# lucianpls/QB3

Measured on AMD Instinct MI355X. Metric: MPixel/s encode+decode (QB3M_FTL, 8-bit 3-band), higher is better.
Workload: dtype u8; 1 GPU; 16384x16384x3 uint8 NOISY3 seed 2; QB3M_FTL qb3x_encode_device (self-indexed container, table level 2) + qb3x_decode_device of that container alone (index = NULL, restart table inside the container); table_level=2, container_bytes=458870207

## Files before the change

qb3_amd/csrc/api_mem.cpp:

```cpp
#include <chrono>
#include <mutex>
#include "qb3_host.h"

using namespace qb3dev;
using namespace qb3api;

struct DevPool {
    struct Item { void *p; size_t cap; int dev; };
    static constexpr size_t POOL_ITEMS = 24;
    const size_t POOL_BYTES = [] { const char *e = getenv("QB3_POOL_MB"); return (e && e[0] ? (size_t)strtoull(e, nullptr, 10) : (size_t)3072) << 20; }();
    std::mutex mu;
    std::vector<Item> items;
    size_t bytes = 0;
    void *take(size_t n, int dev, size_t *cap) {
        std::lock_guard<std::mutex> l(mu);
        size_t best = items.size();
        for (size_t i = 0; i < items.size(); i++)
            if (items[i].dev == dev && items[i].cap >= n && items[i].cap / 2 <= n && (best == items.size() || items[i].cap < items[best].cap)) best = i;
        if (best == items.size()) return nullptr;
        void *p = items[best].p;
        *cap = items[best].cap;
        bytes -= items[best].cap;
        items.erase(items.begin() + (long)best);
        return p;
// ... 46 lines not shown
    bool any = false;
    for (DevBuf *b : bufs) any = any || b->p != nullptr;
    if (any) (void)hipDeviceSynchronize();
    for (DevBuf *b : bufs) b->release(true);
}
QB3_API void qb3x_trim(void) { try { dev_pool().trim(); qb3host::ring_trim(); } catch (...) {} }

bool qb3api::device_ok() {
    int n = 0;
    hipError_t e = hipGetDeviceCount(&n);
    if (e != hipSuccess || n <= 0) { set_error("no usable HIP device (the block codec has no CPU fallback)", (int)e); return false; }
    return true;
}

hipError_t qb3api::wait_stream(hipStream_t st) {
    const auto t0 = std::chrono::steady_clock::now();
    for (uint32_t i = 0;; i++) {
        const hipError_t e = hipStreamQuery(st);
        if (e != hipErrorNotReady) return e;
        if ((i & 63) == 63 && std::chrono::steady_clock::now() - t0 > std::chrono::milliseconds(4)) break;
    }
    return hipStreamSynchronize(st);
}
hipError_t qb3api::fetch_small(void *dst, const void *d_src, size_t n, hipStream_t st) {
    static thread_local void *pinned = nullptr;
    if (!pinned && hipHostMalloc(&pinned, 1024, hipHostMallocDefault) != hipSuccess) pinned = nullptr;
    if (!pinned || n > 1024) {
        hipError_t e = hipMemcpyAsync(dst, d_src, n, hipMemcpyDeviceToHost, st);
        return e == hipSuccess ? hipStreamSynchronize(st) : e;
    }
    hipError_t e = hipMemcpyAsync(pinned, d_src, n, hipMemcpyDeviceToHost, st);
    if (e == hipSuccess) e = wait_stream(st);
    if (e == hipSuccess) memcpy(dst, pinned, n);
    return e;
}

static void parallel_memcpy(uint8_t *dst, const uint8_t *src, size_t n) {
    try { qb3host::CopyPool::get().copy(dst, src, n); }
    catch (...) { memcpy(dst, src, n); }
}
bool qb3api::upload(Stager &sg, void *d_dst, const void *h_src, size_t bytes, hipStream_t st) {
    if (bytes < Stager::MIN_BYTES || !sg.init()) {
        hipError_t e = hipMemcpyAsync(d_dst, h_src, bytes, hipMemcpyHostToDevice, st);
        if (e != hipSuccess) { set_error("upload", (int)e); return false; }
        return true;
    }
    size_t i = 0;
    for (size_t off = 0; off < bytes; off += Stager::SLICE, i++) {
        const size_t n = std::min(Stager::SLICE, bytes - off);
        if (i >= Stager::NSLOT && hipEventSynchronize(sg.ev(i)) != hipSuccess) { set_error("upload: slot wait", 0); return false; }
// ... 60 lines not shown
```

qb3_amd/csrc/api_tiles.cpp:

```cpp
#include "qb3_host.h"

using namespace qb3dev;
using namespace qb3api;

static size_t encode_tiles_loop(encsp p, const void *d_src, size_t first, size_t n, size_t src_pitch, void *d_dst, size_t dst_pitch,
                                void *d_index, size_t isz, size_t *sizes, void *stream, qb3_mode mode) {
    size_t done = 0;
    for (size_t i = first; i < first + n; i++) {
        qb3_reset_encoder(p);
        p->mode = mode;
        sizes[i] = qb3x_encode_device(p, (const uint8_t *)d_src + i * src_pitch, (uint8_t *)d_dst + i * dst_pitch,
                                      d_index ? (uint8_t *)d_index + i * isz : nullptr, stream);
        done += sizes[i] != 0;
    }
    return done;
}

static size_t encode_tiles_body(encsp p, const void *d_src, size_t n, size_t src_pitch, void *d_dst, size_t dst_pitch,
                                void *d_index, size_t *sizes, void *stream) {
    if (!p || !d_src || !d_dst || !sizes || (dst_pitch & 3) || ((uintptr_t)d_dst & 3)) return 0;
    const size_t isz = d_index ? qb3x_index_size(p) : 0;
    const qb3_mode mode = p->mode;
    const size_t tsz = szof(p->type);
    hipStream_t st = (hipStream_t)stream;
    const bool batchable = !is_rle_mode(mode) && mode != QB3M_STORED && p->quanta < 2 && p->xsize >= 4 && p->ysize >= 4 &&
                           p->xsize * p->ysize > 16 && !p->error && device_ok();
    if (!batchable) {
        const size_t k = encode_tiles_loop(p, d_src, 0, n, src_pitch, d_dst, dst_pitch, d_index, isz, sizes, stream, mode);
        if (mode != QB3M_STORED) p->mode = mode;
        return k;
    }

    uint8_t hdrbuf[80];
    size_t hdr = write_headers(p, hdrbuf);
    Geometry g = make_geometry(p->xsize, p->ysize, p->nbands, p->type, p->stride, p->order, p->mode, p->cband, nullptr);
    EncPlan plan = plan_encode(g);
    size_t wsp = (plan.ws_bytes + 255) & ~(size_t)255;
    size_t batch = (size_t)8 << 30 >= wsp ? ((size_t)8 << 30) / wsp : 1;
    if (batch > n) batch = n;
    if (batch > 65535) batch = 65535;
    if (!p->d_ws.ensure(batch * wsp)) { p->error = QB3E_LIBERR; return 0; }
    IxTable ixt;
    size_t hdr_stamp = hdr, ix_bytes = 0, isz_all = isz;
    void *index_all = d_index;
    if (ix_room(p)) {
        ixt = ix_layout(g, p->ix_chunk);
        hdr_stamp = write_headers(p, hdrbuf, false);
// ... 163 lines not shown
```

qb3_amd/csrc/k_enc_post.hip:

```cpp
#include "qb3_kernels.h"
#include "qb3_ix_fill.h"

namespace qb3dev {

__global__ void __launch_bounds__(SCAN_GROUP / 4) enc_scan_kernel(const EncArgs a0) {
    const EncArgs a = enc_for_tile(a0, blockIdx.y);
    __shared__ uint32_t wsum[16];
    __shared__ uint64_t wsum64[16];
    __shared__ uint64_t carry;
    __shared__ uint32_t is_last;
    const uint32_t tid = threadIdx.x, i0 = blockIdx.x * SCAN_GROUP + 4 * tid;
    const uint32_t ngroups = (a.nchunks + SCAN_GROUP - 1) / SCAN_GROUP;
    uint32_t v[4], sum = 0;
#pragma unroll
    for (int k = 0; k < 4; k++) { v[k] = (i0 + k < a.nchunks) ? a.chunk_bits[i0 + k] : 0; sum += v[k]; }
    uint32_t total;
    uint64_t off = block_exscan(sum, wsum, &total);
#pragma unroll
    for (int k = 0; k < 4; k++) if (i0 + k < a.nchunks) { a.chunk_off[i0 + k] = off; off += v[k]; }
    if (tid == 0) {
        a.group_sum[blockIdx.x] = total;
        __threadfence();
        is_last = atomicAdd((uint32_t *)&a.group_sum[ngroups + 1], 1u) == gridDim.x - 1;
        carry = 0;
    }
    __syncthreads();
    if (!is_last) return;
    __threadfence();
    for (uint32_t base = 0; base < ngroups; base += blockDim.x) {
        const uint32_t i = base + tid;
        const uint64_t g = i < ngroups ? __hip_atomic_load(&a.group_sum[i], __ATOMIC_RELAXED, __HIP_MEMORY_SCOPE_AGENT) : 0ull;
        const uint64_t ex = block_exscan_v<uint64_t>(g, wsum64);
        const uint64_t c0 = carry;
        if (i < ngroups) a.group_sum[i] = c0 + ex;
        __syncthreads();
        if (tid == blockDim.x - 1) carry = c0 + ex + g;
        __syncthreads();
    }
    if (tid == 0) { a.group_sum[ngroups] = carry; a.res->zero_run = 0; a.res->ff_pairs = 0; a.res->zero_dwords = 0; }
}

__device__ __forceinline__ uint64_t chunk_start(const EncArgs &a, uint32_t k) {
    if (k >= a.nchunks) return a.group_sum[(a.nchunks + SCAN_GROUP - 1) / SCAN_GROUP];
    return a.group_sum[k / SCAN_GROUP] + a.chunk_off[k];
}

__device__ __forceinline__ uint32_t zero_runs_in(uint32_t cur, uint32_t nxt) {
    return (uint32_t)(cur == 0) + (uint32_t)(__builtin_amdgcn_alignbit(nxt, cur, 8) == 0) +
           (uint32_t)(__builtin_amdgcn_alignbit(nxt, cur, 16) == 0) + (uint32_t)(__builtin_amdgcn_alignbit(nxt, cur, 24) == 0);
}
__device__ __forceinline__ uint32_t ff_pairs_in(uint32_t v) {
    const uint32_t t = v & (v >> 8) & 0x00ffffffu;
    return (uint32_t)__popc(((t & 0x7f7f7fu) + 0x010101u) & t & 0x808080u);
}

__device__ __forceinline__ void ix_finish_chunk(const EncArgs &a, uint32_t c) {
    typedef uint32_t u32_a1 __attribute__((aligned(1)));
    __shared__ uint32_t part[4];
    const uint32_t tid = threadIdx.x;
    const uint32_t here = (a.ix_K - c * a.ix_per_chunk < a.ix_per_chunk) ? a.ix_K - c * a.ix_per_chunk : a.ix_per_chunk;
    uint8_t *chunk = a.ix_dst + (uint64_t)c * (IX_HEAD + IX_PAD + (uint64_t)a.ix_per_chunk * a.ix_E);
    uint8_t *e0 = chunk + IX_HEAD;
// ... 318 lines not shown
```

qb3_amd/csrc/k_host.hip:

```cpp
#include "qb3_kernels.h"
#include "qb3_walk.h"

namespace qb3dev {

static thread_local char g_err[256] = "";
const char *last_error() { return g_err; }
void set_error(const char *what, int e) {
    snprintf(g_err, sizeof(g_err), "%s: %s", what, e ? hipGetErrorString((hipError_t)e) : "failed");
}

const Tuning &tuning() {
    static const Tuning t = [] {
        auto on = [](const char *name) { const char *e = getenv(name); return e && e[0] && e[0] != '0'; };
        Tuning v;
        v.no_px = on("QB3_NO_PX");
        v.slow_walk = on("QB3_SLOW_WALK");
        const char *cap = getenv("QB3_WALK_TAB_KB");
        v.walk_tab_kb = cap ? (size_t)strtoull(cap, nullptr, 10) : 0;
        v.slow_index = on("QB3_SLOW_INDEX");
        { const char *e = getenv("QB3_WIDE_BAND"); v.wide_band = e && e[0] ? atoi(e) : 0; }
        v.no_bl = on("QB3_NO_BLOCK_LENGTHS");
        { const char *e = getenv("QB3_BEST_SAMPLE_MIN"); v.best_sample_min = e && e[0] ? (uint32_t)strtoul(e, nullptr, 10) : BEST_SAMPLE_MIN; }
        { const char *e = getenv("QB3_EXITS_FROM"); v.exits_from = e && e[0] ? (int64_t)strtoll(e, nullptr, 10) : -1; }
        return v;
    }();
    return t;
}

}
#include <map>
#include <mutex>
#include <string>
#include <vector>
namespace qb3dev {
struct ProfPending { const char *name; hipEvent_t a, b; };
static std::mutex g_prof_mu;
static int g_prof_level = 0;
static std::vector<ProfPending> g_prof_pending;
static std::vector<hipEvent_t> g_prof_pool;
static std::map<std::string, std::pair<double, uint64_t>> g_prof_acc;
void prof_enable(int level) { std::lock_guard<std::mutex> l(g_prof_mu); g_prof_level = level; }
static bool prof_minor(const char *n) { const std::string s(n); return s == "enc_scan" || s == "enc_seams" || s == "enc_best_scan" || s == "enc_best_recode"; }
void prof_reset() { std::lock_guard<std::mutex> l(g_prof_mu); g_prof_acc.clear(); }
static hipEvent_t prof_event() {
    if (!g_prof_pool.empty()) { hipEvent_t e = g_prof_pool.back(); g_prof_pool.pop_back(); return e; }
    hipEvent_t e = nullptr;
    (void)hipEventCreate(&e);
    return e;
}
ProfScope::ProfScope(const char *n, hipStream_t s) : st(s), name(n) {
    std::lock_guard<std::mutex> l(g_prof_mu);
    on = g_prof_level == 1 || (g_prof_level == 2 && !prof_minor(n)) || (g_prof_level >= 3 && std::string(n).find("_units") != std::string::npos);
    if (on) { a = prof_event(); b = prof_event(); (void)hipEventRecord(a, st); }
}
ProfScope::~ProfScope() {
    if (!on) return;
    (void)hipEventRecord(b, st);
    std::lock_guard<std::mutex> l(g_prof_mu);
    g_prof_pending.push_back({name, a, b});
}
void prof_collect() {
    std::lock_guard<std::mutex> l(g_prof_mu);
    std::vector<ProfPending> keep;
    for (auto &p : g_prof_pending) {
        float ms = 0;
        const hipError_t e = hipEventElapsedTime(&ms, p.a, p.b);
        if (e == hipErrorNotReady) { keep.push_back(p); continue; }
        if (e == hipSuccess) { auto &acc = g_prof_acc[p.name]; acc.first += ms; acc.second++; }
        g_prof_pool.push_back(p.a); g_prof_pool.push_back(p.b);
    }
    (void)hipGetLastError();
    g_prof_pending.swap(keep);
}
bool prof_get(const char *name, double *total_ms, uint64_t *count) {
    std::lock_guard<std::mutex> l(g_prof_mu);
    auto it = g_prof_acc.find(name);
    if (it == g_prof_acc.end()) return false;
    *total_ms = it->second.first; *count = it->second.second;
    return true;
}
int prof_names(char *buf, size_t n) {
    std::lock_guard<std::mutex> l(g_prof_mu);
    std::string s;
    for (auto &kv : g_prof_acc) { if (!s.empty()) s += ","; s += kv.first; }
    snprintf(buf, n, "%s", s.c_str());
    return (int)g_prof_acc.size();
}


static void fast_geometry(uint32_t bands, uint32_t tsz, uint32_t *threads, uint32_t *bpp, uint32_t *passes) {
    *threads = tsz == 8 ? 128 : 256;
    *bpp = *threads / bands;
    uint32_t k = (uint32_t)(16384 / ((size_t)*bpp * bands * tsz * 16));
    *passes = k < 1 ? 1 : (k > 3 ? 3 : k);
}
static void px16_split(const Geometry &g, uint32_t *bg, uint32_t *ng) {
    const uint32_t B = g.bands;
    *bg = B <= 4 ? B : (B % 4 == 0) ? 4 : (B % 2 == 0) ? 2 : 0;
    *ng = *bg ? B / *bg : 0;
}
uint32_t px16_bands_per_lane(const Geometry &g) { uint32_t bg, ng; px16_split(g, &bg, &ng); return bg; }

uint32_t seg_blocks_for(const Geometry &g) {
    if (lane_per_unit_shape(g.tsz, g.mode, g.bands)) return 64 / g.bands;
    if (g.mode != CM_BEST) {
// ... 175 lines not shown
}

static void launch_enc_units(const EncArgs &a, const EncPlan &plan, hipStream_t st) {
    if (a.g.mode == CM_BEST) { if (plan.px && a.g.tsz == 1) launch_enc_px_best(a, plan, st); else launch_enc_best(a, plan, st); }
    else if (plan.px && a.g.tsz == 1) {
        ProfScope ps("enc_units", st);
        launch_enc_px(a, plan, st);
    }
    else if (plan.px16 && a.g.tsz == 2 && ((uintptr_t)a.img & 1) == 0) { ProfScope ps("enc_units", st); launch_enc_px16(a, plan, st); }
    else if (plan.pxw && ((uintptr_t)a.img & (a.g.tsz - 1)) == 0 && !(a.ts_img & (a.g.tsz - 1))) { ProfScope ps("enc_units", st); launch_enc_pxw(a, plan, st); }
    else { ProfScope ps("enc_units", st); launch_enc_generic(a, plan, st); }
}
static int launch_encode_all(const EncArgs &a, const EncPlan &plan, hipStream_t st) {
    launch_enc_units(a, plan, st);
    launch_enc_post(a, plan, st);
    HIPCHK(hipGetLastError());
    return 0;
}

static bool make_enc_args(EncArgs &a, const Geometry &g, const EncPlan &plan, const void *img, uint32_t *out32, uint32_t out_bit0,
                          const BandState &st_in, void *ws, void *index, const TileBatch &tb,
                          const uint8_t *hdr, uint32_t hdr_len, const IxTable &ix, bool zrun_probe) {
    a.zrun_probe = zrun_probe ? 1u : 0u;
    a.ix_dst = ix.base; a.ix_K = ix.K; a.ix_E = ix.entry_bytes; a.ix_per_chunk = ix.per_chunk; a.ix_blocks = ix.blocks;
    a.ix_spe = g.seg_blocks ? ix.blocks / g.seg_blocks : 0;
    a.ntiles = tb.n ? tb.n : 1; a.ts_img = tb.src_pitch; a.ts_out = tb.dst_pitch; a.ts_ws = tb.ws_pitch; a.ts_idx = tb.idx_pitch;
    a.hdr_len = hdr_len <= sizeof(a.hdr) ? hdr_len : 0;
    a.hdr_back = a.hdr_len + (ix.base ? (uint32_t)ix_total_bytes(ix) + 2 : 0);
    for (uint32_t i = 0; i < a.hdr_len; i++) a.hdr[i] = hdr[i];
    a.g = g; a.img = img; a.out32 = out32; a.out_bit0 = out_bit0;
    a.slots = plan.slots; a.nchunks = plan.nchunks; a.dpr = g.bands * g.tsz;
    a.chunk0 = 0; a.chunk_end = plan.nchunks; a.finish_what = 3;
    a.magic_dpr = magic_div(a.dpr); a.magic_bands = magic_div(g.bands);
    uint8_t *w = (uint8_t *)ws;
    const EncWs L = enc_ws_layout(g, plan.nchunks, plan.nbp, plan.threads);
    a.chunk_bits = (uint32_t *)(w + L.bits);
    a.chunk_off = (uint64_t *)(w + L.off);
    a.group_sum = (uint64_t *)(w + L.gsum);
    a.seams = (uint32_t *)(w + L.seams);
    a.scratch = (uint32_t *)(w + L.scratch);
    a.cw_has = w + L.cwhas; a.cw_val = (uint64_t *)(w + L.cwval); a.centry = (uint64_t *)(w + L.centry); a.centry_parts = (uint32_t *)(w + L.cparts); a.recode_n = a.centry_parts + 32 * MAXBANDS;
    a.cw_used = w + L.cwused; a.seg_from_entry = w + L.segfe; a.recode_need = (uint32_t *)(w + L.rneed); a.recode_list = (uint32_t *)(w + L.rlist);
    a.slot_dw = L.slot_dw;
    a.px_ng = plan.px16 ? plan.px16_ng : 1; a.px_magic_ng = magic_div(a.px_ng);
    a.px16_bg = g.tsz == 2 ? px16_bands_per_lane(g) : 0;
    a.px_aligned = !(g.w & 3) && !((g.stride * g.tsz) & 3) && !((uintptr_t)img & 3) && !(tb.src_pitch & 3);
    a.res = (EncResult *)(w + L.res);
    a.st = st_in;
    a.ix_bl = ix.base && ix.block_lens;
    a.ix_coder = a.ix_bl && plan.px && g.tsz == 1 && g.mode != CM_BEST && g.seg_blocks == 64 && ix.blocks == 64;
    a.ix_wgs = 0;
    a.have_idx = index != nullptr && !(a.ix_coder && ix.own_index);
    a.idx_no_ulen = index && ix.base && ix.own_index && !ix.block_lens;
    a.idx = index ? index_view(g, index) : IndexView{nullptr, nullptr, nullptr, nullptr, nullptr};
    if (g.tsz != 1 && g.tsz != 2 && g.tsz != 4 && g.tsz != 8) { set_error("encode: bad value size", 0); return false; }
    return true;
}

int launch_encode(const Geometry &g, const EncPlan &plan, const void *img, uint32_t *out32, uint32_t out_bit0,
                  const BandState &st_in, void *ws, void *index, void *stream, const TileBatch &tb,
                  const uint8_t *hdr, uint32_t hdr_len, const IxTable &ix, bool zrun_probe) {
    EncArgs a;
    if (!make_enc_args(a, g, plan, img, out32, out_bit0, st_in, ws, index, tb, hdr, hdr_len, ix, zrun_probe)) return -1;
    return launch_encode_all(a, plan, (hipStream_t)stream);
}

bool encode_strips_ok(const Geometry &g, const EncPlan &plan) { return g.mode != CM_BEST && plan.nchunks > 2 * SCAN_GROUP; }
uint32_t encode_strip_count(const EncPlan &plan) { return (plan.nchunks + SCAN_GROUP - 1) / SCAN_GROUP; }
uint64_t encode_strip_blocks(const EncPlan &plan, uint32_t strip) {
    const uint64_t c = std::min<uint64_t>(plan.nchunks, ((uint64_t)strip + 1) * SCAN_GROUP);
    return c * plan.nbp;
}
const uint64_t *encode_strip_total(const Geometry &g, const EncPlan &plan, void *ws, uint32_t strip) {
    const EncWs L = enc_ws_layout(g, plan.nchunks, plan.nbp, plan.threads);
    return (const uint64_t *)((uint8_t *)ws + L.gsum) + strip + 1;
}
int launch_encode_strip(const Geometry &g, const EncPlan &plan, const void *img, uint32_t *out32, uint32_t out_bit0,
                        const BandState &st_in, void *ws, void *index, void *stream, const uint8_t *hdr, uint32_t hdr_len, const IxTable &ix, uint32_t strip) {
    EncArgs a;
    if (!make_enc_args(a, g, plan, img, out32, out_bit0, st_in, ws, index, TileBatch(), hdr, hdr_len, ix, false)) return -1;
    a.chunk0 = strip * SCAN_GROUP;
    a.chunk_end = std::min<uint32_t>(plan.nchunks, a.chunk0 + SCAN_GROUP);
    a.finish_what = 1;
    hipStream_t st = (hipStream_t)stream;
    launch_enc_units(a, plan, st);
    launch_enc_post_strip(a, plan, st, strip);
// ... 152 lines not shown
```

qb3_amd/csrc/qb3_api.cpp:

```cpp
#include <chrono>
#include <new>
#include <limits>
#include <thread>
#include "qb3_host.h"

using namespace qb3dev;
using namespace qb3api;

static size_t raw_size(const encs *p) { return p->xsize * p->ysize * p->nbands * szof(p->type); }

static CodecMode codec_mode(int mode) {
    if (mode == QB3M_FTL) return CM_FTL;
    if (mode == QB3M_BASE_H || mode == QB3M_BASE_Z || mode == QB3M_RLE || mode == QB3M_RLE_H) return CM_BASE;
    return CM_BEST;
}

Geometry qb3api::make_geometry(size_t w, size_t h, size_t bands, int dtype, size_t stride, uint64_t order, int mode,
                              const size_t *cband_sz, const uint8_t *cband_u8) {
    Geometry g;
    memset(&g, 0, sizeof(g));
    g.w = (uint32_t)w; g.h = (uint32_t)h; g.bands = (uint32_t)bands; g.tsz = (uint32_t)szof(dtype);
    g.stride = stride ? stride : w * bands;
    g.order = order ? order : HILBERT;
    g.nbx = (uint32_t)((w + 3) / 4); g.nby = (uint32_t)((h + 3) / 4);
// ... 87 lines not shown
    if (w < 4) {
        for (size_t y = 0; y < h; y++, d += w * pix) memcpy(d, src + y * stride_bytes, w * pix);
        nw = 4; nh = ngroups * 4;
    } else {
        for (size_t x = 0; x < w; x++)
            for (size_t y = 0; y < h; y++, d += pix) memcpy(d, src + y * stride_bytes + x * pix, pix);
        nw = ngroups * 4; nh = 4;
    }
    return t;
}


static size_t stored_encode_host(encsp p, const void *source, void *destination) {
    uint8_t *d = (uint8_t *)destination;
    p->mode = QB3M_STORED;
    const size_t hdr = write_headers(p, d);
    if (p->error) return 0;
    const size_t tsz = szof(p->type), line = p->xsize * p->nbands * tsz;
    const size_t stride = (p->stride ? p->stride : p->xsize * p->nbands) * tsz;
    for (size_t y = 0; y < p->ysize; y++) memcpy(d + hdr + y * line, (const uint8_t *)source + y * stride, line);
    return hdr + raw_size(p);
}

static bool encode_blocks_device(encsp p, const Geometry &g, const void *d_img, uint8_t *d_out, size_t hdr,
                                 void *d_index, hipStream_t st, bool carry, uint64_t *bits, const uint8_t *hdrbytes,
                                 size_t hdr_stamp, const IxTable &ix, int *zero_run = nullptr) {
    EncPlan plan = plan_encode(g);
    if (!p->d_ws.ensure(plan.ws_bytes)) return false;
    BandState bs;
    memset(&bs, 0, sizeof(bs));
    for (size_t c = 0; c < p->nbands; c++) {
        bs.prev[c] = p->band[c].prev; bs.cf[c] = p->band[c].cf; bs.rung[c] = (uint8_t)p->band[c].runbits;
    }
    uint32_t *out32 = (uint32_t *)(d_out + (hdr & ~(size_t)3));
    EncResult res;
    const uint8_t *dres = (const uint8_t *)p->d_ws.p + plan.ws_bytes - sizeof(EncResult);
    if (launch_encode(g, plan, d_img, out32, (uint32_t)(8 * (hdr & 3)), bs, p->d_ws.p, d_index, st, TileBatch(), hdrbytes, (uint32_t)hdr_stamp, ix, zero_run != nullptr)) return false;
    const hipError_t e = fetch_small(&res, dres, sizeof(res), st);
    if (e != hipSuccess) { set_error("encode kernels", (int)e); return false; }
    prof_collect();
    *bits = res.total_bits;
    { static const bool dbg = getenv("QB3_DEBUG_RLE") != nullptr; if (dbg && zero_run) fprintf(stderr, "encode: zero_run %llu ff_pairs %llu zero_dwords %llu (%u chunks)\n", (unsigned long long)res.zero_run, (unsigned long long)res.ff_pairs, (unsigned long long)res.zero_dwords, plan.nchunks); }
    if (zero_run) *zero_run = rle0_may_win(res) ? (rle0_no_uniform_chunk(res, (uint64_t)plan.nbp * g.bands / 4) ? 2 : 1) : 0;
    if (carry)
        for (size_t c = 0; c < p->nbands; c++) {
            p->band[c].prev = (size_t)res.prev[c]; p->band[c].runbits = res.rung[c]; p->band[c].cf = (size_t)res.cf[c];
        }
    return true;
}

struct ModeGuard {
    encs *p; qb3_mode mode; bool armed = true;
    ModeGuard(encs *h) : p(h), mode(h->mode) {}
    ~ModeGuard() { if (armed) p->mode = mode; }
};


static int encode_pipelined(encsp p, const Geometry &g, const void *host_src, void *host_dst, size_t src_bytes, size_t line, uint8_t *out_dev, size_t hdr,
                            const uint8_t *hdrbuf, size_t hdr_stamp, const IxTable &ixt, void *d_index, bool carry, uint64_t *bits_out) {
    using qb3host::CopyPool;
    constexpr size_t SLICE = Stager::SLICE, NSLOT = Stager::NSLOT;
    static const bool dbg = getenv("QB3_DEBUG_PIPE") != nullptr;
// ... 87 lines not shown
            if (q == hipSuccess) { if (dbg && !dn_copy) t_first_dn = ms_since(); pool.submit(dn[dn_copy].host, r2.slot(dn_copy), dn[dn_copy].n, b_dn[dn_copy % NSLOT]); dn_copy++; progress = true; }
            else if (q != hipErrorNotReady) e = q;
        }
        while (dn_freed < dn_copy && pool.done(b_dn[dn_freed % NSLOT])) { dn_freed++; progress = true; }
        if (!progress && !pool.help_one()) std::this_thread::yield();
    }
    (void)hipGetLastError();
    for (size_t i = 0; i < NSLOT; i++) { pool.wait(b_up[i]); pool.wait(b_dn[i]); }
    p->pipe.sync();
    if (dbg) fprintf(stderr, "encode_pipelined: setup %.2f ms, last upload enqueued %.2f, first slice down %.2f, done %.2f (%u strips, %zu + %zu slices)\n", t_setup, t_up_done, t_first_dn, ms_since(), nstrips, n_up, dn.size());
    if (!ok()) { if (!launch_failed) set_error("pipelined encode", (int)e); p->error = QB3E_LIBERR; return -1; }
    prof_collect();
    *bits_out = res_host->total_bits;
    if (carry)
        for (size_t c = 0; c < p->nbands; c++) {
            p->band[c].prev = (size_t)res_host->prev[c]; p->band[c].runbits = res_host->rung[c]; p->band[c].cf = (size_t)res_host->cf[c];
        }
    return 1;
}

static size_t encode_common(encsp p, const void *host_src, void *host_dst, const void *d_src, void *d_dst,
                            void *d_index, hipStream_t st) {
    const bool on_host = host_src != nullptr;
    const size_t tsz = szof(p->type), line = p->xsize * p->nbands * tsz;
    const size_t src_stride_bytes = (p->stride ? p->stride : p->xsize * p->nbands) * tsz;
    const size_t src_span = src_stride_bytes * (p->ysize - 1) + line;
    if (p->xsize * p->ysize <= 16) {
        if (on_host) return stored_encode_host(p, host_src, host_dst);
        std::vector<uint8_t> tmp(src_span), out(64 + raw_size(p));
        if (!device_ok()) { p->error = QB3E_LIBERR; return 0; }
        HIPOK(hipMemcpyAsync(tmp.data(), d_src, tmp.size(), hipMemcpyDeviceToHost, st));
        HIPOK(hipStreamSynchronize(st));
        size_t n = stored_encode_host(p, tmp.data(), out.data());
        HIPOK(hipMemcpyAsync(d_dst, out.data(), n, hipMemcpyHostToDevice, st));
        HIPOK(hipStreamSynchronize(st));
        return n;
    }
    ModeGuard guard(p);
    const qb3_mode mode = p->mode;
    const bool rle = is_rle_mode(mode);
    const size_t ixroom = mode == QB3M_STORED ? 0 : ix_room(p);
    if (rle) p->mode = (qb3_mode)((int)mode - 2);
    uint8_t hdrbuf[80];
    size_t hdr = write_headers(p, hdrbuf);
    if (p->error) return 0;
    if (!device_ok()) { p->error = QB3E_LIBERR; return 0; }
// ... 44 lines not shown

    IxTable ixt;
    size_t hdr_stamp = hdr;
    if (ixroom && !narrow) {
        ixt = ix_layout(g, p->ix_chunk);
        hdr_stamp = write_headers(p, hdrbuf, false);
        hdr = hdr_stamp + ix_total_bytes(ixt) + 2;
        ixt.base = out_dev + hdr_stamp;
        if (!d_index) {
            if (!p->d_idx.ensure(index_bytes(g))) { p->error = QB3E_LIBERR; return 0; }
            d_index = p->d_idx.p;
            ixt.own_index = true;
        }
    }
    uint64_t bits = 0;
    int has_run = 1;
    bool piped = false;
    if (want_pipe) {
        const int r = encode_pipelined(p, g, host_src, host_dst, src_span, line, out_dev, hdr, hdrbuf, hdr_stamp, ixt, d_index, carry, &bits);
        if (r < 0) return 0;
        piped = r > 0;
        if (!piped && !upload_now()) { p->error = QB3E_LIBERR; return 0; }
    }
    if (!piped && !encode_blocks_device(p, g, img_dev, out_dev, hdr, d_index, st, carry, &bits, hdrbuf, hdr_stamp, ixt, rle ? &has_run : nullptr)) {
        p->error = QB3E_LIBERR; return 0;
    }
    p->error = 0;
    const size_t len = hdr + (size_t)((bits + 7) / 8);
    const size_t len_ref = len - (ixt.base ? ix_total_bytes(ixt) : 0);

    if (rle) {
        p->mode = mode;
        if (len_ref <= maxsz / 2 && has_run) {
            const size_t n = len - hdr;
            uint64_t rsz64 = 0;
            if (!p->d_rle.ensure(rle0_ws_bytes(n)) || rle0_device_size(out_dev + hdr, n, p->d_rle.p, false, &rsz64, st, has_run == 2)) { p->error = QB3E_LIBERR; return 0; }
            const size_t rsz = (size_t)rsz64;
            if (rsz <= maxsz - len_ref && rsz < n) {
                uint8_t hdr2[80];
                const size_t tbl = ixt.base ? hdr - hdr_stamp : 0;
                const size_t h2 = write_headers(p, hdr2, tbl == 0);
                if (!p->d_q.ensure(rsz) || rle0_device_write(out_dev + hdr, n, p->d_rle.p, false, p->d_q.p, st)) { p->error = QB3E_LIBERR; return 0; }
                if (on_host) {
                    memcpy(host_dst, hdr2, h2);
                    if (tbl && !download(p->stager, (uint8_t *)host_dst + h2, out_dev + hdr_stamp, tbl, st)) { p->error = QB3E_LIBERR; return 0; }
                    if (!download(p->stager, (uint8_t *)host_dst + h2 + tbl, p->d_q.p, rsz, st)) { p->error = QB3E_LIBERR; return 0; }
                } else {
// ... 382 lines not shown
```

qb3_amd/csrc/qb3_dev.h:

```cpp
#pragma once
#include <stddef.h>
#include <stdint.h>
#include <algorithm>
#include <vector>

namespace qb3dev {

constexpr int MAXBANDS = 16;
constexpr uint64_t ZCURVE = 0x0145236789cdabefull;
constexpr uint64_t HILBERT = 0x01548cd9aefb7623ull;

enum CodecMode { CM_FTL = 0, CM_BASE = 1, CM_BEST = 2 };

struct Geometry {
    uint32_t w, h, bands, tsz;
    uint64_t stride;
    uint64_t order;
    uint32_t nbx, nby;
    uint64_t nblocks;
    uint32_t mode;
    uint32_t seg_blocks;
    uint64_t nseg;
    uint32_t ulen_sz;
    uint8_t cband[MAXBANDS];
// ... 24 lines not shown
}

inline bool lane_per_unit_shape(uint32_t tsz, uint32_t mode, uint32_t bands) {
    if (bands < 1 || bands > (uint32_t)MAXBANDS) return false;
    if (mode == CM_BEST) return !best_block_table(tsz, mode, bands);
    if (tsz == 1) return !(bands == 1 || bands == 3 || bands == 4);
    if (tsz == 2) return bands > 4 && (bands & 1);
    return bands >= 2;
}

constexpr uint64_t WIN_LAUNCH_WAVES = 1ull << 24;
inline bool window_unit_geometry_ok(const Geometry &g) {
    return g.seg_blocks && (uint64_t)g.nby * (g.nbx / g.seg_blocks + 2) <= WIN_LAUNCH_WAVES && g.nblocks < (1ull << 31);
}

struct EncResult {
    uint64_t total_bits;
    uint64_t prev[MAXBANDS];
    uint64_t cf[MAXBANDS];
    uint32_t rung[MAXBANDS];
    uint64_t zero_run;
    uint64_t ff_pairs;
    uint64_t zero_dwords;
};

inline bool rle0_may_win(const EncResult &r) { return r.zero_run > 0 && 2 * r.zero_run + 2 > r.ff_pairs; }
inline bool rle0_no_uniform_chunk(const EncResult &r, uint64_t min_chunk_bytes) {
    if (min_chunk_bytes < 16) return false;
    const uint64_t shared = 2 * (4096 / min_chunk_bytes + 2);
    return shared < 1000 && r.zero_dwords < 1022 - shared && r.ff_pairs < 1024;
}

struct EncPlan {
    uint32_t threads;
    uint32_t slots;
    uint32_t nchunks;
    size_t lds_bytes;
    size_t ws_bytes;
    uint32_t nbp;
    bool px;
    bool px_rgb;
    bool px16;
    uint32_t px16_bg, px16_ng;
    bool pxw;
    bool pxw_best;
};
// ... 22 lines not shown
inline uint32_t ix_bl_bytes(uint32_t tsz, uint32_t bands, uint32_t blocks, bool cf) {
    const bool per_unit = lane_per_unit_shape(tsz, cf ? CM_BEST : CM_FTL, bands);
    if (cf) return IX_BL_BEST_BYTES * blocks * (per_unit ? bands : 1u);
    if (per_unit) return (blocks * bands * IX_BL_BITS_WIDE + 7) / 8;
    const uint32_t fields = tsz == 1 ? blocks : tsz == 2 ? (bands == 1 ? 64u : 128u) : blocks * bands;
    return (fields * ix_bl_bits(tsz) + 7) / 8;
}
IxTable ix_layout(const Geometry &g, int level = 1);
inline size_t ix_chunks(const IxTable &t) { return t.per_chunk ? (t.K + t.per_chunk - 1) / t.per_chunk : 0; }
inline size_t ix_total_bytes(const IxTable &t) { return ix_chunks(t) * (IX_HEAD + (t.pads ? IX_PAD : 0)) + (size_t)t.K * t.entry_bytes; }

struct TileBatch { uint32_t n = 0; uint64_t src_pitch = 0, dst_pitch = 0, ws_pitch = 0, idx_pitch = 0; uint64_t max_bits = 0;  };
size_t walk_table_bytes(uint32_t ntiles, uint64_t max_bits, uint32_t tsz);
size_t walk_table_min_bytes(uint32_t ntiles, uint32_t tsz);
size_t walk_memory_bytes(const Geometry &g, uint32_t ntiles, uint64_t max_bits);
size_t walk_table_cap();
struct DecPlan;
bool walk_table_applies(const Geometry &g, const DecPlan &plan);

int launch_encode(const Geometry &g, const EncPlan &plan, const void *img, uint32_t *out32, uint32_t out_bit0,
                  const BandState &st_in, void *ws, void *index, void *stream, const TileBatch &tb = TileBatch(),
                  const uint8_t *hdr = nullptr, uint32_t hdr_len = 0,
                  const IxTable &ix = IxTable(),
                  bool zrun_probe = false);

bool encode_strips_ok(const Geometry &g, const EncPlan &plan);
uint32_t encode_strip_count(const EncPlan &plan);
uint64_t encode_strip_blocks(const EncPlan &plan, uint32_t strip);
const uint64_t *encode_strip_total(const Geometry &g, const EncPlan &plan, void *ws, uint32_t strip);
int launch_encode_strip(const Geometry &g, const EncPlan &plan, const void *img, uint32_t *out32, uint32_t out_bit0,
                        const BandState &st_in, void *ws, void *index, void *stream, const uint8_t *hdr, uint32_t hdr_len, const IxTable &ix, uint32_t strip);
int launch_encode_tail(const Geometry &g, const EncPlan &plan, const void *img, uint32_t *out32, uint32_t out_bit0,
                       const BandState &st_in, void *ws, void *index, void *stream, const uint8_t *hdr, uint32_t hdr_len, const IxTable &ix);

struct DecPlan {
    uint32_t threads;
    uint32_t nwg;
    size_t lds_bytes;
    size_t ws_bytes;
    bool fast;
    uint32_t threads2, bpp, passes, in_cap_dw;
    size_t lds2_bytes;
    bool px, px_rgb;
    size_t lds_px;
    uint32_t px_cap_dw;
    bool px16;
    uint32_t px16_bg, px16_ng;
// ... 93 lines not shown
```

qb3_amd/csrc/qb3_host.h:

```cpp
#pragma once
#include <hip/hip_runtime_api.h>
#include <cstring>
#include <cstdlib>
#include <cstdio>
#include <exception>
#include <initializer_list>
#include <vector>
#include <utility>
#include <algorithm>
#include "../../include/QB3.h"
#include "../../include/qb3x.h"
#include "qb3_dev.h"
#include "qb3_host_io.h"

#define QB3_API extern "C" __attribute__((visibility("default")))
#define HIPOK(x) do { hipError_t e_ = (x); if (e_ != hipSuccess) { qb3dev::set_error(#x, (int)e_); p->error = QB3E_LIBERR; return 0; } } while (0)

struct DevBuf {
    void *p = nullptr;
    size_t cap = 0;
    int dev = 0;
    bool ensure(size_t n);
    void release(bool idle = false);
};
// ... 32 lines not shown
    static constexpr size_t WORDS = 2048;
    bool failed = false;
    bool init();
    bool events(size_t n);
    void sync() { if (up) { (void)hipStreamSynchronize(up); (void)hipStreamSynchronize(k); (void)hipStreamSynchronize(dn); } }
    void release();
};

struct band_state { size_t prev, runbits, cf; };

struct encs {
    size_t xsize, ysize, nbands, stride;
    uint64_t order, quanta;
    band_state band[QB3_MAXBANDS];
    size_t cband[QB3_MAXBANDS];
    int error;
    qb3_mode mode;
    qb3_dtype type;
    bool away;
    int ix_chunk;
    DevBuf d_img, d_out, d_ws, d_q, d_idx, d_rle;
    Stager stager, stager2;
    Pipe pipe;
};

struct decs {
    size_t xsize, ysize, nbands, stride;
    uint64_t order, quanta;
    int error, stage;
    uint8_t cband[QB3_MAXBANDS];
    qb3_mode mode;
    qb3_dtype type;
    uint8_t *s_in;
    size_t s_size;
    uint8_t *s_start;
    bool saw_cb;
    unsigned compat;
    size_t hdr_avail;
    size_t ix_off;
    uint32_t ix_K, ix_blocks, ix_E, ix_per_chunk;
    bool ix_bl;
    bool ix_pads, ix_bad;
    uint32_t ix_ver;
    bool ix_heads_unchecked;
    bool hdr_short;
    size_t ix_need_off;
// ... 19 lines not shown
    PinBuf h_rg;
    DevBuf d_rg;
};

namespace qb3api {

inline size_t szof(int dt) {
    constexpr int typesizes[8] = { 1, 1, 2, 2, 4, 4, 8, 8 };
    return (dt < 0 || dt > QB3_I64) ? 0 : typesizes[dt];
}
inline bool is_rle_mode(int m) { return m == QB3M_RLE || m == QB3M_CF_RLE || m == QB3M_RLE_H || m == QB3M_CF_RLE_H; }

template <class R, class F> R abi_guard(R fail, F &&f) noexcept {
    try { return f(); }
    catch (const std::exception &e) { qb3dev::set_error(e.what(), -1); }
    catch (...) { qb3dev::set_error("C++ exception inside the library", -1); }
    return fail;
}

void release_all(std::initializer_list<DevBuf *> bufs);
bool device_ok();
hipError_t wait_stream(hipStream_t st);
hipError_t fetch_small(void *dst, const void *d_src, size_t n, hipStream_t st);
bool upload(Stager &sg, void *d_dst, const void *h_src, size_t bytes, hipStream_t st);
bool download(Stager &sg, void *h_dst, const void *d_src, size_t bytes, hipStream_t st);

size_t write_headers(const encs *p, uint8_t *dst, bool with_dt = true);
decsp read_start_impl(void *source, size_t hdr_avail, size_t source_size, size_t *image_size);
qb3dev::IxTable handle_table(const decs *p, const uint8_t *base);
qb3dev::Geometry decoder_geometry(const decs *p, size_t w, size_t h, size_t stride);

inline size_t win_stride(const decs *p, const qb3x_window &w) { return w.dst_stride ? w.dst_stride : w.w * p->nbands; }
inline bool window_inside(const decs *p, size_t x0, size_t y0, size_t w, size_t h) {
    return w && h && x0 < p->xsize && w <= p->xsize - x0 && y0 < p->ysize && h <= p->ysize - y0;
}
template <class T> inline void merge_ranges(std::vector<std::pair<T, T>> &r, T gap = 0) {
    std::sort(r.begin(), r.end());
    size_t m = 0;
    for (size_t i = 1; i < r.size(); i++) {
        if (r[i].first - std::min(r[i].first, r[m].second) <= gap) r[m].second = std::max(r[m].second, r[i].second);
        else r[++m] = r[i];
    }
    if (!r.empty()) r.resize(m + 1);
}
inline const qb3dev::WinKernels *family_if_aligned(const qb3dev::WinKernels *fam, const qb3dev::Geometry &g, const qb3x_window *wins, size_t n) {
    for (size_t i = 0; fam && i < n; i++) if ((uintptr_t)wins[i].dst & (fam->align(g) - 1)) fam = nullptr;
// ... 17 lines not shown
```

qb3_amd/csrc/qb3_kernels.h:

```cpp
#pragma once
#include <hip/hip_runtime.h>
#include <algorithm>
#include <type_traits>
#include "qb3_dev.h"

namespace qb3dev {

template <typename T> struct UBits { static constexpr uint32_t v = sizeof(T) == 1 ? 3 : sizeof(T) == 2 ? 4 : sizeof(T) == 4 ? 5 : 6; };

template <typename T> __device__ __forceinline__ T mags_t(T v) {
    constexpr uint32_t B = 8 * sizeof(T);
    return (T)((T)(v << 1) ^ (T)(0 - (T)(v >> (B - 1))));
}
template <typename T> __device__ __forceinline__ T smag_t(T v) {
    return (T)((T)(v >> 1) ^ (T)(0 - (T)(v & 1)));
}
template <typename T> __device__ __forceinline__ T mabs_t(T v) { return (T)((v >> 1) + (v & 1)); }
template <typename T> __device__ __forceinline__ T mmul_t(T v, T m) { return (T)((T)(mabs_t<T>(v) * (T)(m << 1)) - (T)(v & 1)); }
__device__ __forceinline__ uint32_t topbit64(uint64_t v) { return 63u - (uint32_t)__clzll((long long)v); }
__device__ __forceinline__ uint32_t topbit32(uint32_t v) { return 31u - (uint32_t)__clz((int)v); }
template <typename T> __device__ __forceinline__ uint32_t topbit_t(T v) {
    if (sizeof(T) == 8) return topbit64((uint64_t)v | 1);
    return topbit32((uint32_t)v | 1);
}
// ... 138 lines not shown
    uint32_t *recode_need, *recode_list, *recode_n;
    uint32_t ntiles;
    uint64_t ts_img, ts_out, ts_ws, ts_idx;
    uint32_t hdr_len;
    uint32_t hdr_back;
    uint8_t hdr[80];
    uint32_t px_ng, px_magic_ng;
    uint32_t px16_bg;
    uint32_t px_aligned;
    uint8_t *ix_dst;
    uint32_t ix_K, ix_spe, ix_E;
    uint32_t ix_bl;
    uint32_t ix_per_chunk, ix_blocks;
    uint32_t ix_coder;
    uint32_t ix_wgs;
    EncResult *res;
    BandState st;
    IndexView idx;
    uint32_t have_idx;
    uint32_t zrun_probe;
    uint32_t idx_no_ulen;
    uint32_t chunk0, chunk_end;
    uint32_t finish_what;
};


template <typename P> __device__ __forceinline__ P *shift_ptr(P *p, uint64_t bytes) { return p ? (P *)((uint8_t *)p + bytes) : p; }
__device__ __forceinline__ EncArgs enc_for_tile(EncArgs a, uint32_t t) {
    if (t) {
        a.img = (const uint8_t *)a.img + t * a.ts_img;
        a.out32 = shift_ptr(a.out32, t * a.ts_out);
        const uint64_t w = t * a.ts_ws, x = t * a.ts_idx;
        a.chunk_bits = shift_ptr(a.chunk_bits, w); a.chunk_off = shift_ptr(a.chunk_off, w); a.group_sum = shift_ptr(a.group_sum, w);
        a.scratch = shift_ptr(a.scratch, w); a.seams = shift_ptr(a.seams, w); a.res = shift_ptr(a.res, w);
        a.cw_has = shift_ptr(a.cw_has, w); a.cw_val = shift_ptr(a.cw_val, w); a.centry = shift_ptr(a.centry, w); a.cw_used = shift_ptr(a.cw_used, w); a.seg_from_entry = shift_ptr(a.seg_from_entry, w); a.recode_need = shift_ptr(a.recode_need, w); a.recode_list = shift_ptr(a.recode_list, w); a.recode_n = shift_ptr(a.recode_n, w); a.centry_parts = shift_ptr(a.centry_parts, w);
        a.idx.bitpos = shift_ptr(a.idx.bitpos, x); a.idx.prev = shift_ptr(a.idx.prev, x); a.idx.cf = shift_ptr(a.idx.cf, x);
        a.idx.rung = shift_ptr(a.idx.rung, x); a.idx.ulen = shift_ptr(a.idx.ulen, x);
        a.ix_dst = shift_ptr(a.ix_dst, t * a.ts_out);
    }
    return a;
}

struct LdsWriter {
    uint32_t *buf;
    uint64_t acc;
    uint32_t n, w;
// ... 363 lines not shown
```

Measured before the change: 312,800 MPixel/s.

## Return from device encode early via mapped host block before tail kernels finish

After the group-sum scan the encode kernel writes total bits and per-band state into a mapped, coherent host block and publishes a sequence number. The host polls that word and returns as soon as it appears, instead of waiting on the stream for the full result fetch. The remaining tail kernels keep running, and the encoder records a pending tail that is synchronized on the next call that uses a different stream or host buffers. The profiler also gains generation tagging and lazy resolution. The risk is that callers on the same stream are relied on for ordering, and system-scope stores add some kernel cost.

```diff
diff --git a/qb3_amd/csrc/api_mem.cpp b/qb3_amd/csrc/api_mem.cpp
--- a/qb3_amd/csrc/api_mem.cpp
+++ b/qb3_amd/csrc/api_mem.cpp
@@ -92,10 +92,34 @@
     }
     return hipStreamSynchronize(st);
 }
+namespace {
+constexpr size_t FETCH_BYTES = 1024;
+struct HostBlock { void *host = nullptr; void *dev = nullptr; int device = -1; bool tried = false; uint64_t seq = 0; };
+HostBlock &host_block() {
+    static thread_local HostBlock b;
+    if (!b.tried) {
+        b.tried = true;
+        if (hipHostMalloc(&b.host, FETCH_BYTES + sizeof(EncEarly), hipHostMallocMapped | hipHostMallocCoherent) != hipSuccess) { (void)hipGetLastError(); b.host = nullptr; }
+        if (b.host) {
+            memset(b.host, 0, FETCH_BYTES + sizeof(EncEarly));
+            if (hipGetDevice(&b.device) != hipSuccess || hipHostGetDevicePointer(&b.dev, b.host, 0) != hipSuccess) { (void)hipGetLastError(); b.dev = nullptr; }
+        }
+    }
+    return b;
+}
+}
+bool qb3api::host_early_block(volatile EncEarly **host, EncEarly **dev, uint64_t *seq) {
+    HostBlock &b = host_block();
+    int cur = -1;
+    if (!b.host || !b.dev || hipGetDevice(&cur) != hipSuccess || cur != b.device) return false;
+    *host = (volatile EncEarly *)((uint8_t *)b.host + FETCH_BYTES);
+    *dev = (EncEarly *)((uint8_t *)b.dev + FETCH_BYTES);
+    *seq = ++b.seq;
+    return true;
+}
 hipError_t qb3api::fetch_small(void *dst, const void *d_src, size_t n, hipStream_t st) {
-    static thread_local void *pinned = nullptr;
-    if (!pinned && hipHostMalloc(&pinned, 1024, hipHostMallocDefault) != hipSuccess) pinned = nullptr;
-    if (!pinned || n > 1024) {
+    void *pinned = host_block().host;
+    if (!pinned || n > FETCH_BYTES) {
         hipError_t e = hipMemcpyAsync(dst, d_src, n, hipMemcpyDeviceToHost, st);
         return e == hipSuccess ? hipStreamSynchronize(st) : e;
     }
diff --git a/qb3_amd/csrc/api_tiles.cpp b/qb3_amd/csrc/api_tiles.cpp
--- a/qb3_amd/csrc/api_tiles.cpp
+++ b/qb3_amd/csrc/api_tiles.cpp
@@ -6,6 +6,7 @@
 static size_t encode_tiles_loop(encsp p, const void *d_src, size_t first, size_t n, size_t src_pitch, void *d_dst, size_t dst_pitch,
                                 void *d_index, size_t isz, size_t *sizes, void *stream, qb3_mode mode) {
     size_t done = 0;
+    struct Hold { encs *p; bool was; Hold(encs *h) : p(h), was(h->hold_tail) { h->hold_tail = true; } ~Hold() { p->hold_tail = was; } } hold(p);
     for (size_t i = first; i < first + n; i++) {
         qb3_reset_encoder(p);
         p->mode = mode;
@@ -23,6 +24,7 @@
     const qb3_mode mode = p->mode;
     const size_t tsz = szof(p->type);
     hipStream_t st = (hipStream_t)stream;
+    p->settle_tail(st);
     const bool batchable = !is_rle_mode(mode) && mode != QB3M_STORED && p->quanta < 2 && p->xsize >= 4 && p->ysize >= 4 &&
                            p->xsize * p->ysize > 16 && !p->error && device_ok();
     if (!batchable) {
diff --git a/qb3_amd/csrc/k_enc_post.hip b/qb3_amd/csrc/k_enc_post.hip
--- a/qb3_amd/csrc/k_enc_post.hip
+++ b/qb3_amd/csrc/k_enc_post.hip
@@ -38,6 +38,20 @@
         __syncthreads();
     }
     if (tid == 0) { a.group_sum[ngroups] = carry; a.res->zero_run = 0; a.res->ff_pairs = 0; a.res->zero_dwords = 0; }
+    if (a.early) {
+        EncEarly *h = a.early;
+        if (tid == 0) __hip_atomic_store(&h->total_bits, (uint64_t)carry, __ATOMIC_RELAXED, __HIP_MEMORY_SCOPE_SYSTEM);
+        if (tid < a.g.bands && tid < (uint32_t)MAXBANDS) {
+            const uint64_t pv = a.res->prev[tid], cf = a.res->cf[tid];
+            const uint32_t rg = a.res->rung[tid];
+            __hip_atomic_store(&h->prev[tid], pv, __ATOMIC_RELAXED, __HIP_MEMORY_SCOPE_SYSTEM);
+            __hip_atomic_store(&h->cf[tid], cf, __ATOMIC_RELAXED, __HIP_MEMORY_SCOPE_SYSTEM);
+            __hip_atomic_store(&h->rung[tid], rg, __ATOMIC_RELAXED, __HIP_MEMORY_SCOPE_SYSTEM);
+        }
+        __threadfence_system();
+        __syncthreads();
+        if (tid == 0) __hip_atomic_store(&h->seq, a.early_seq, __ATOMIC_RELEASE, __HIP_MEMORY_SCOPE_SYSTEM);
+    }
 }
 
 __device__ __forceinline__ uint64_t chunk_start(const EncArgs &a, uint32_t k) {
diff --git a/qb3_amd/csrc/k_host.hip b/qb3_amd/csrc/k_host.hip
--- a/qb3_amd/csrc/k_host.hip
+++ b/qb3_amd/csrc/k_host.hip
@@ -33,13 +33,14 @@
 #include <string>
 #include <vector>
 namespace qb3dev {
-struct ProfPending { const char *name; hipEvent_t a, b; };
+struct ProfPending { const char *name; hipEvent_t a, b; uint64_t gen; };
 static std::mutex g_prof_mu;
 static int g_prof_level = 0;
+static uint64_t g_prof_gen = 0;
 static std::vector<ProfPending> g_prof_pending;
 static std::vector<hipEvent_t> g_prof_pool;
 static std::map<std::string, std::pair<double, uint64_t>> g_prof_acc;
-void prof_enable(int level) { std::lock_guard<std::mutex> l(g_prof_mu); g_prof_level = level; }
+void prof_enable(int level) { std::lock_guard<std::mutex> l(g_prof_mu); if (!g_prof_level && level) g_prof_gen++; g_prof_level = level; }
 static bool prof_minor(const char *n) { const std::string s(n); return s == "enc_scan" || s == "enc_seams" || s == "enc_best_scan" || s == "enc_best_recode"; }
 void prof_reset() { std::lock_guard<std::mutex> l(g_prof_mu); g_prof_acc.clear(); }
 static hipEvent_t prof_event() {
@@ -57,23 +58,25 @@
     if (!on) return;
     (void)hipEventRecord(b, st);
     std::lock_guard<std::mutex> l(g_prof_mu);
-    g_prof_pending.push_back({name, a, b});
-}
-void prof_collect() {
-    std::lock_guard<std::mutex> l(g_prof_mu);
+    g_prof_pending.push_back({name, a, b, g_prof_gen});
+}
+static void prof_resolve() {
+    if (g_prof_pending.empty()) return;
     std::vector<ProfPending> keep;
     for (auto &p : g_prof_pending) {
         float ms = 0;
         const hipError_t e = hipEventElapsedTime(&ms, p.a, p.b);
         if (e == hipErrorNotReady) { keep.push_back(p); continue; }
-        if (e == hipSuccess) { auto &acc = g_prof_acc[p.name]; acc.first += ms; acc.second++; }
+        if (e == hipSuccess && p.gen == g_prof_gen) { auto &acc = g_prof_acc[p.name]; acc.first += ms; acc.second++; }
         g_prof_pool.push_back(p.a); g_prof_pool.push_back(p.b);
     }
     (void)hipGetLastError();
     g_prof_pending.swap(keep);
 }
+void prof_collect() { std::lock_guard<std::mutex> l(g_prof_mu); prof_resolve(); }
 bool prof_get(const char *name, double *total_ms, uint64_t *count) {
     std::lock_guard<std::mutex> l(g_prof_mu);
+    prof_resolve();
     auto it = g_prof_acc.find(name);
     if (it == g_prof_acc.end()) return false;
     *total_ms = it->second.first; *count = it->second.second;
@@ -81,6 +84,7 @@
 }
 int prof_names(char *buf, size_t n) {
     std::lock_guard<std::mutex> l(g_prof_mu);
+    prof_resolve();
     std::string s;
     for (auto &kv : g_prof_acc) { if (!s.empty()) s += ","; s += kv.first; }
     snprintf(buf, n, "%s", s.c_str());
@@ -302,6 +306,7 @@
                           const BandState &st_in, void *ws, void *index, const TileBatch &tb,
                           const uint8_t *hdr, uint32_t hdr_len, const IxTable &ix, bool zrun_probe) {
     a.zrun_probe = zrun_probe ? 1u : 0u;
+    a.early = nullptr; a.early_seq = 0;
     a.ix_dst = ix.base; a.ix_K = ix.K; a.ix_E = ix.entry_bytes; a.ix_per_chunk = ix.per_chunk; a.ix_blocks = ix.blocks;
     a.ix_spe = g.seg_blocks ? ix.blocks / g.seg_blocks : 0;
     a.ntiles = tb.n ? tb.n : 1; a.ts_img = tb.src_pitch; a.ts_out = tb.dst_pitch; a.ts_ws = tb.ws_pitch; a.ts_idx = tb.idx_pitch;
@@ -339,9 +344,10 @@
 
 int launch_encode(const Geometry &g, const EncPlan &plan, const void *img, uint32_t *out32, uint32_t out_bit0,
                   const BandState &st_in, void *ws, void *index, void *stream, const TileBatch &tb,
-                  const uint8_t *hdr, uint32_t hdr_len, const IxTable &ix, bool zrun_probe) {
+                  const uint8_t *hdr, uint32_t hdr_len, const IxTable &ix, bool zrun_probe, EncEarly *early, uint64_t early_seq) {
     EncArgs a;
     if (!make_enc_args(a, g, plan, img, out32, out_bit0, st_in, ws, index, tb, hdr, hdr_len, ix, zrun_probe)) return -1;
+    if (!tb.n && !zrun_probe && g.mode != CM_BEST) { a.early = early; a.early_seq = early_seq; }
     return launch_encode_all(a, plan, (hipStream_t)stream);
 }
 
diff --git a/qb3_amd/csrc/qb3_api.cpp b/qb3_amd/csrc/qb3_api.cpp
--- a/qb3_amd/csrc/qb3_api.cpp
+++ b/qb3_amd/csrc/qb3_api.cpp
@@ -1,3 +1,4 @@
+#include <atomic>
 #include <chrono>
 #include <new>
 #include <limits>
@@ -133,9 +134,39 @@
     return hdr + raw_size(p);
 }
 
+static bool early_return_off() {
+    static const bool off = [] { const char *e = getenv("QB3_NO_EARLY_RETURN"); return e && e[0] && e[0] != '0'; }();
+    return off;
+}
+struct EarlyCount {
+    std::atomic<uint64_t> early{0}, late{0}, fell_back{0}, wait_us{0};
+    const bool dbg = getenv("QB3_DEBUG_EARLY") != nullptr;
+    ~EarlyCount() {
+        if (dbg) fprintf(stderr, "encode early return: %llu calls returned with the tail in flight, %llu saw the word once the stream was done, %llu fell back to the stream wait; %llu us polling\n",
+                         (unsigned long long)early.load(), (unsigned long long)late.load(), (unsigned long long)fell_back.load(), (unsigned long long)wait_us.load());
+    }
+};
+static EarlyCount g_early_count;
+static int wait_early(volatile EncEarly *blk, uint64_t seq, size_t nbands, hipStream_t st, EncResult *res) {
+    const auto t0 = std::chrono::steady_clock::now();
+    bool seen = false, done = false;
+    for (uint32_t i = 0; !seen; i++) {
+        seen = __atomic_load_n(&blk->seq, __ATOMIC_ACQUIRE) == seq;
+        if (seen || (i & 63) != 63) continue;
+        const hipError_t q = hipStreamQuery(st);
+        if (q != hipErrorNotReady) { done = true; seen = q == hipSuccess && __atomic_load_n(&blk->seq, __ATOMIC_ACQUIRE) == seq; break; }
+        if (std::chrono::steady_clock::now() - t0 > std::chrono::milliseconds(4)) break;
+    }
+    (void)hipGetLastError();
+    if (g_early_count.dbg) g_early_count.wait_us += (uint64_t)std::chrono::duration_cast<std::chrono::microseconds>(std::chrono::steady_clock::now() - t0).count();
+    if (!seen) return 0;
+    res->total_bits = blk->total_bits;
+    for (size_t c = 0; c < nbands; c++) { res->prev[c] = blk->prev[c]; res->cf[c] = blk->cf[c]; res->rung[c] = blk->rung[c]; }
+    return done ? 2 : 1;
+}
 static bool encode_blocks_device(encsp p, const Geometry &g, const void *d_img, uint8_t *d_out, size_t hdr,
                                  void *d_index, hipStream_t st, bool carry, uint64_t *bits, const uint8_t *hdrbytes,
-                                 size_t hdr_stamp, const IxTable &ix, int *zero_run = nullptr) {
+                                 size_t hdr_stamp, const IxTable &ix, int *zero_run = nullptr, bool early = false) {
     EncPlan plan = plan_encode(g);
     if (!p->d_ws.ensure(plan.ws_bytes)) return false;
     BandState bs;
@@ -145,10 +176,23 @@
     }
     uint32_t *out32 = (uint32_t *)(d_out + (hdr & ~(size_t)3));
     EncResult res;
+    memset(&res, 0, sizeof(res));
     const uint8_t *dres = (const uint8_t *)p->d_ws.p + plan.ws_bytes - sizeof(EncResult);
-    if (launch_encode(g, plan, d_img, out32, (uint32_t)(8 * (hdr & 3)), bs, p->d_ws.p, d_index, st, TileBatch(), hdrbytes, (uint32_t)hdr_stamp, ix, zero_run != nullptr)) return false;
-    const hipError_t e = fetch_small(&res, dres, sizeof(res), st);
-    if (e != hipSuccess) { set_error("encode kernels", (int)e); return false; }
+    volatile EncEarly *blk = nullptr;
+    EncEarly *blk_dev = nullptr;
+    uint64_t seq = 0;
+    early = early && !zero_run && g.mode != CM_BEST && !p->hold_tail && !early_return_off() && host_early_block(&blk, &blk_dev, &seq);
+    if (launch_encode(g, plan, d_img, out32, (uint32_t)(8 * (hdr & 3)), bs, p->d_ws.p, d_index, st, TileBatch(), hdrbytes, (uint32_t)hdr_stamp, ix, zero_run != nullptr,
+                      early ? blk_dev : nullptr, seq)) return false;
+    const int got = early ? wait_early(blk, seq, p->nbands, st, &res) : 0;
+    if (got) {
+        p->tail_pending = got == 1; p->tail_stream = st;
+        (got == 1 ? g_early_count.early : g_early_count.late)++;
+    } else {
+        if (early) g_early_count.fell_back++;
+        const hipError_t e = fetch_small(&res, dres, sizeof(res), st);
+        if (e != hipSuccess) { set_error("encode kernels", (int)e); return false; }
+    }
     prof_collect();
     *bits = res.total_bits;
     { static const bool dbg = getenv("QB3_DEBUG_RLE") != nullptr; if (dbg && zero_run) fprintf(stderr, "encode: zero_run %llu ff_pairs %llu zero_dwords %llu (%u chunks)\n", (unsigned long long)res.zero_run, (unsigned long long)res.ff_pairs, (unsigned long long)res.zero_dwords, plan.nchunks); }
@@ -282,6 +326,7 @@
 static size_t encode_common(encsp p, const void *host_src, void *host_dst, const void *d_src, void *d_dst,
                             void *d_index, hipStream_t st) {
     const bool on_host = host_src != nullptr;
+    p->settle_tail(st, on_host);
     const size_t tsz = szof(p->type), line = p->xsize * p->nbands * tsz;
     const size_t src_stride_bytes = (p->stride ? p->stride : p->xsize * p->nbands) * tsz;
     const size_t src_span = src_stride_bytes * (p->ysize - 1) + line;
@@ -372,7 +417,7 @@
         piped = r > 0;
         if (!piped && !upload_now()) { p->error = QB3E_LIBERR; return 0; }
     }
-    if (!piped && !encode_blocks_device(p, g, img_dev, out_dev, hdr, d_index, st, carry, &bits, hdrbuf, hdr_stamp, ixt, rle ? &has_run : nullptr)) {
+    if (!piped && !encode_blocks_device(p, g, img_dev, out_dev, hdr, d_index, st, carry, &bits, hdrbuf, hdr_stamp, ixt, rle ? &has_run : nullptr, !on_host)) {
         p->error = QB3E_LIBERR; return 0;
     }
     p->error = 0;
diff --git a/qb3_amd/csrc/qb3_dev.h b/qb3_amd/csrc/qb3_dev.h
--- a/qb3_amd/csrc/qb3_dev.h
+++ b/qb3_amd/csrc/qb3_dev.h
@@ -70,6 +70,14 @@
     uint64_t zero_run;
     uint64_t ff_pairs;
     uint64_t zero_dwords;
+};
+
+struct EncEarly {
+    uint64_t total_bits;
+    uint64_t prev[MAXBANDS];
+    uint64_t cf[MAXBANDS];
+    uint32_t rung[MAXBANDS];
+    uint64_t seq;
 };
 
 inline bool rle0_may_win(const EncResult &r) { return r.zero_run > 0 && 2 * r.zero_run + 2 > r.ff_pairs; }
@@ -138,7 +146,8 @@
                   const BandState &st_in, void *ws, void *index, void *stream, const TileBatch &tb = TileBatch(),
                   const uint8_t *hdr = nullptr, uint32_t hdr_len = 0,
                   const IxTable &ix = IxTable(),
-                  bool zrun_probe = false);
+                  bool zrun_probe = false,
+                  EncEarly *early = nullptr, uint64_t early_seq = 0);
 
 bool encode_strips_ok(const Geometry &g, const EncPlan &plan);
 uint32_t encode_strip_count(const EncPlan &plan);
diff --git a/qb3_amd/csrc/qb3_host.h b/qb3_amd/csrc/qb3_host.h
--- a/qb3_amd/csrc/qb3_host.h
+++ b/qb3_amd/csrc/qb3_host.h
@@ -78,6 +78,13 @@
     DevBuf d_img, d_out, d_ws, d_q, d_idx, d_rle;
     Stager stager, stager2;
     Pipe pipe;
+    bool tail_pending = false;
+    hipStream_t tail_stream = nullptr;
+    bool hold_tail = false;
+    void settle_tail(hipStream_t st, bool other_streams = false) {
+        if (tail_pending && (other_streams || st != tail_stream)) { (void)hipStreamSynchronize(tail_stream); (void)hipGetLastError(); }
+        tail_pending = false;
+    }
 };
 
 struct decs {
@@ -143,6 +150,7 @@
 bool device_ok();
 hipError_t wait_stream(hipStream_t st);
 hipError_t fetch_small(void *dst, const void *d_src, size_t n, hipStream_t st);
+bool host_early_block(volatile qb3dev::EncEarly **host, qb3dev::EncEarly **dev, uint64_t *seq);
 bool upload(Stager &sg, void *d_dst, const void *h_src, size_t bytes, hipStream_t st);
 bool download(Stager &sg, void *h_dst, const void *d_src, size_t bytes, hipStream_t st);
 
diff --git a/qb3_amd/csrc/qb3_kernels.h b/qb3_amd/csrc/qb3_kernels.h
--- a/qb3_amd/csrc/qb3_kernels.h
+++ b/qb3_amd/csrc/qb3_kernels.h
@@ -184,6 +184,8 @@
     uint32_t idx_no_ulen;
     uint32_t chunk0, chunk_end;
     uint32_t finish_what;
+    EncEarly *early;
+    uint64_t early_seq;
 };
 
 
```

Result: no change. 314,300 MPixel/s, median of 6 (+0.5%).
